# XiaoshuiHuang/GMF

Hardware: AMD Instinct MI355X
Metric: correspondences/sec (whole node) (higher is better)
Workload: dtype f32 (split-fp16 MFMA operands, fp32 accumulate; the cross products of the attention's two contractions, S = K Q'^T and O = P V, on block-scaled e4m3 operands wherever the device-side score guard allows)

## Files before the change

gmf_amd/csrc/enc_common.hpp:

```cpp
#pragma once
#include "mfma_core.hpp"
#include "launchers.hpp"

namespace gmf {

constexpr int C = 128;
constexpr int CF = C / 2;
constexpr int DH = 64;
constexpr int DHF = DH / 2;
constexpr int FFH = 512;
constexpr int kWavesPerWG = 4;

GMF_DEVINL void load_vec_block(float (&v)[16], const float* __restrict__ vec, int mb, int h) {
  const float4* p = reinterpret_cast<const float4*>(vec + 32 * mb) + h;
#pragma unroll
  for (int q = 0; q < 4; ++q) {
    const float4 t = p[2 * q];
    v[4 * q + 0] = t.x; v[4 * q + 1] = t.y; v[4 * q + 2] = t.z; v[4 * q + 3] = t.w;
  }
}

GMF_DEVINL void store_block_p32(float* __restrict__ tile_base, int mb, const float (&t)[16], int lane) {
  float4* p = reinterpret_cast<float4*>(tile_base) + (4 * mb) * 64 + lane;
#pragma unroll
  for (int q = 0; q < 4; ++q) p[q * 64] = make_float4(t[4 * q + 0], t[4 * q + 1], t[4 * q + 2], t[4 * q + 3]);
}

GMF_DEVINL void load_block_p32(float (&t)[16], const float* __restrict__ tile_base, int mb, int lane) {
  const float4* p = reinterpret_cast<const float4*>(tile_base) + (4 * mb) * 64 + lane;
#pragma unroll
  for (int q = 0; q < 4; ++q) {
    const float4 v = p[q * 64];
    t[4 * q + 0] = v.x; t[4 * q + 1] = v.y; t[4 * q + 2] = v.z; t[4 * q + 3] = v.w;
  }
}

GMF_DEVINL void store_block_timg(float* __restrict__ tile_base, int db, const f32x16& a, float bias, int lane) {
  float4* p = reinterpret_cast<float4*>(tile_base) + (4 * db) * 64 + lane;
#pragma unroll
  for (int q = 0; q < 4; ++q)
    p[q * 64] = make_float4(a[4 * q + 0] + bias, a[4 * q + 1] + bias, a[4 * q + 2] + bias, a[4 * q + 3] + bias);
}

GMF_DEVINL void store_block_h2(float* __restrict__ tile_base, int blk, const float (&t)[16], int lane) {
  f16x8* base = reinterpret_cast<f16x8*>(tile_base);
#pragma unroll
  for (int half = 0; half < 2; ++half) {
    f16x8 hi, lo;
    split8h(&t[8 * half], hi, lo);
    const int slot = 2 * blk + half;
    base[(0 * 8 + slot) * 64 + lane] = hi;
    base[(1 * 8 + slot) * 64 + lane] = lo;
  }
}

GMF_DEVINL void store_block_v8(float* __restrict__ tile_base, int db, const float (&t)[16], int lane, unsigned& scale_word) {
  f16x8* base = reinterpret_cast<f16x8*>(tile_base);
  float mx = 0.f;
#pragma unroll
  for (int r = 0; r < 16; ++r) mx = __builtin_fmaxf(mx, __builtin_fabsf(t[r]));
  mx = xhalf_max_swap(mx);
  const int e = (int)((__float_as_uint(mx) >> 23) & 0xffu);
  const int sb = max(e - 7, 105);
  const float s_hi = __uint_as_float((unsigned)sb << 23), s_lo = __uint_as_float((unsigned)(sb - 11) << 23);
  scale_word |= (unsigned)((lane & 32) ? sb : sb - 11) << (8 * db);
  i32x4 v8, l8;
#pragma unroll
  for (int half = 0; half < 2; ++half) {
    f16x8 hi;
#pragma unroll
    for (int j = 0; j < 8; j += 2) {
      const float x0 = t[8 * half + j], x1 = t[8 * half + j + 1];
      const f32x2 x = {x0, x1};
      const f16x2 hh = __builtin_convertvector(x, f16x2);
      const f32x2 rl = resid2h(hh, x0, x1);
      hi[j] = hh[0]; hi[j + 1] = hh[1];
      const int w = 2 * half + (j >> 2);
      if (j & 2) { v8[w] = cvt2_fp8_f32<true>(v8[w], x0, x1, s_hi); l8[w] = cvt2_fp8_f32<true>(l8[w], rl[0], rl[1], s_lo); }
      else { v8[w] = cvt2_fp8_f32<false>(0, x0, x1, s_hi); l8[w] = cvt2_fp8_f32<false>(0, rl[0], rl[1], s_lo); }
    }
    base[(0 * 8 + 2 * db + half) * 64 + lane] = hi;
  }
  reinterpret_cast<i32x4*>(tile_base)[(1 * 8 + 2 * db) * 64 + lane] = l8;
  reinterpret_cast<i32x4*>(tile_base)[(1 * 8 + 2 * db + 1) * 64 + lane] = v8;
}

GMF_DEVINL void q_planes8(const f16x8& h0, const f16x8& l0, const f16x8& h1, const f16x8& l1, int cb, int lane, i32x8& out,
                          unsigned& scale_word) {
  float q[16], ql[16];
#pragma unroll
  for (int e = 0; e < 8; ++e) {
    ql[e] = (float)l0[e]; q[e] = (float)h0[e] + ql[e];
    ql[8 + e] = (float)l1[e]; q[8 + e] = (float)h1[e] + ql[8 + e];
  }
  float mx = 0.f;
#pragma unroll
  for (int r = 0; r < 16; ++r) mx = __builtin_fmaxf(mx, __builtin_fabsf(q[r]));
  mx = xhalf_max_swap(mx);
  const int e = (int)((__float_as_uint(mx) >> 23) & 0xffu);
  const int sb = max(e - 7, 105);
  const float s_hi = __uint_as_float((unsigned)sb << 23), s_lo = __uint_as_float((unsigned)(sb - 11) << 23);
  scale_word |= (unsigned)((lane & 32) ? sb - 11 : sb) << (8 * cb);
#pragma unroll
  for (int w = 0; w < 4; ++w) {
    int a = cvt2_fp8_f32<false>(0, q[4 * w], q[4 * w + 1], s_hi);
    out[w] = cvt2_fp8_f32<true>(a, q[4 * w + 2], q[4 * w + 3], s_hi);
    int b = cvt2_fp8_f32<false>(0, ql[4 * w], ql[4 * w + 1], s_lo);
    out[4 + w] = cvt2_fp8_f32<true>(b, ql[4 * w + 2], ql[4 * w + 3], s_lo);
  }
}

GMF_DEVINL bool pv_planes_on(const unsigned* __restrict__ v_scale, const PvGuard& g, int pair) {
  if (!v_scale) return false;
  if (!g.stat) return true;
// ... 284 lines not shown
```

gmf_amd/csrc/encoder_h2.hip:

```cpp
#include <algorithm>
#include <cstdlib>
#include "enc_common.hpp"
#include "enc_ff.hpp"
#include "launchers.hpp"

namespace gmf {

#ifndef GMF_H2_RING
#define GMF_H2_RING 2
#endif
constexpr int kRing = GMF_H2_RING;

template <int MODE>
GMF_DEVINL void front_h2_body(float* lds, const int bx, const int pair, const int zsel_in, const float* __restrict__ in,
                              const float* __restrict__ wst, const float* __restrict__ vecs, float* __restrict__ f_out,
                              float* __restrict__ q_out, float* __restrict__ k_out, float* __restrict__ v_out, int N, int tiles,
                              const PairTab* __restrict__ ptab = nullptr, unsigned* __restrict__ v_scale = nullptr,
                              const PvGuard guard = {}) {
  const int lane = threadIdx.x & 63, h = lane >> 5, i = lane & 31;
  const int wave = __builtin_amdgcn_readfirstlane(threadIdx.x >> 6);
  const size_t row0 = pair_row0(ptab, pair, N);
  N = pair_rows(ptab, pair, N);
  const int tiles_p = ptab ? (N + 31) >> 5 : tiles;
  if (bx * kWavesPerWG >= tiles_p) return;
// ... 623 lines not shown
  else if (PART != 2) dma_vec(front_vec + C, lvec_p, 3 * C, wave, kWavesPerWG, lane);
  if (PART != 1) {
    dma_vec(attn_vec, lvec_a, 7 * C, wave, kWavesPerWG, lane);
    dma_vec(ff_vec, lvec_f, 3 * C + 2 * FFH, wave, kWavesPerWG, lane);
    LcpeHalo<CF>::issue(pair_base, tile, tiles_p, halo, lane);
  }
  StageRing<4> ss;
  if (KVF && PART == 1) ss.init(lds, wave, lane, kvf_wst, 4);
  else if (KVF && QSKIP) ss.init(lds, wave, lane, attn_wst, 2, ctx_img + (size_t)pair * ttiles * kStageFloats, ttiles, attn_wst + 2 * kStageFloats, 2);
  else if (KVF) ss.init(lds, wave, lane, kvf_wst, 4, attn_wst, 2, ctx_img + (size_t)pair * ttiles * kStageFloats, ttiles, attn_wst + 2 * kStageFloats, 2);
  else if (PART == 0) ss.init(lds, wave, lane, front_wst + (QSKIP ? 8 : 4) * kStageFloats, QSKIP ? 8 : 12, attn_wst, 2,
                         ctx_img + (size_t)pair * ttiles * kStageFloats, ttiles, attn_wst + 2 * kStageFloats, 2);
  else if (PART == 1) ss.init(lds, wave, lane, front_wst + 4 * kStageFloats, 12);
  else ss.init(lds, wave, lane, attn_wst, 2, ctx_img + (size_t)pair * ttiles * kStageFloats, ttiles, attn_wst + 2 * kStageFloats, 2);

  float f[CF];
  if (PART != 2) {
    FragH2<8> fx;
    load_frag_p32<CF>(f, f_in + toff, lane);
    fx.set(f);
    ss.prime();
    const bool v8 = pv_planes_on(v_scale, guard, pair);
    unsigned* const sw_tile = v_scale ? v_scale + ((size_t)pair * tiles + tile) * 128 + lane : nullptr;
    unsigned ksw = 0, vsw = 0;
    if (KVF) {
      asm volatile("s_waitcnt vmcnt(12)" ::: "memory");
      __syncthreads();
      float* const mt = lds + 3 * kStageFloats + wave * 1024;
#pragma unroll
      for (int mb = 0; mb < 4; ++mb) {
        float t[16], td[16];
#pragma unroll
        for (int r = 0; r < 16; ++r) t[r] = f[16 * mb + r];
        if (v8) store_block_v8(k_out + toff, mb, t, lane, ksw);
        else store_block_h2(k_out + toff, mb, t, lane);
#pragma unroll
        for (int r = 0; r < 16; ++r) mt[i * 32 + (frag_feature(r, h) ^ i)] = t[r];
        asm volatile("s_waitcnt lgkmcnt(0)" ::: "memory");
#pragma unroll
        for (int r = 0; r < 16; ++r) { const int kk = frag_feature(r, h); td[r] = mt[kk * 32 + (i ^ kk)]; }
        asm volatile("s_waitcnt lgkmcnt(0)" ::: "memory");
        if (v8) store_block_v8(v_out + toff, mb, td, lane, vsw);
        else store_block_h2(v_out + toff, mb, td, lane);
      }
      if (v_scale) { sw_tile[0] = vsw; sw_tile[64] = ksw; }
      if (!QSKIP) {
#pragma unroll
        for (int mb = 0; mb < 4; ++mb) {
          const f16x8* lw = as_h2(ss.acquire());
          f32x16 acc = zero16();
          mma_wx_h2n<8, NP>(acc, lw, fx);
          float t[16], bb[16];
          load_vec_block(bb, lvec_p, mb, h);
#pragma unroll
          for (int r = 0; r < 16; ++r) t[r] = fmaf(acc[r], kH2Inv, bb[r]);
          store_block_h2(q_out + toff, mb, t, lane);
        }
      }
    }
#pragma unroll
    for (int which = (KVF ? 2 : QSKIP ? 1 : 0); which < 2; ++which) {
      float* dst = (which == 0 ? q_out : k_out) + toff;
#pragma unroll
      for (int mb = 0; mb < 4; ++mb) {
        constexpr int kYounger[4] = {8, 12, 16, 20};
        const int sidx = 4 * (which - (QSKIP ? 1 : 0)) + mb;
        const f16x8* lw = as_h2(PART == 1 ? ss.acquire()
                                : sidx == 0 ? ss.acquire_counted<kYounger[0]>() : sidx == 1 ? ss.acquire_counted<kYounger[1]>()
                                : sidx == 2 ? ss.acquire_counted<kYounger[2]>() : ss.acquire_counted<kYounger[3]>());
        f32x16 acc = zero16();
        mma_wx_h2n<8, NP>(acc, lw, fx);
        float t[16], bb[16];
        load_vec_block(bb, lvec_p + which * C, mb, h);
#pragma unroll
        for (int r = 0; r < 16; ++r) t[r] = fmaf(acc[r], kH2Inv, bb[r]);
// ... 15 lines not shown
    }
    if (v_scale && !KVF) { sw_tile[0] = vsw; sw_tile[64] = ksw; }
  }

  if (PART == 1) {
    asm volatile("s_waitcnt vmcnt(0)" ::: "memory");
    return;
  }
  if (PART == 2) ss.prime();
  f32x16 x1a[4];
  {
    FragH2<4> qx;
    {
      float xp[CF];
      if (PART == 2) load_frag_p32<CF>(xp, f_in + toff, lane);
      else {
#pragma unroll
        for (int k = 0; k < CF; ++k) xp[k] = f[k];
      }
      if (PART == 2) {
        asm volatile("s_waitcnt vmcnt(0)" ::: "memory");
        __syncthreads();
      }
      LcpeHalo<CF>::apply(xp, halo, lvec_a, tile * 32 + i, N, lane);
      {
        FragH2<8> nx;
        {
          float xn[CF];
          layernorm_frag<CF>(xn, xp, lvec_a + 4 * C, lvec_a + 5 * C, h);
          nx.set(xn);
        }
#pragma unroll
        for (int mb = 0; mb < 2; ++mb) {
          const f16x8* lw = as_h2((KVF && QSKIP && PART == 0) ? ss.acquire_counted<40>() : ss.acquire());
          f32x16 acc = zero16();
          mma_wx_h2n<8, NP>(acc, lw, nx);
          float t[16];
#pragma unroll
          for (int r = 0; r < 16; ++r) t[r] = acc[r] * kH2Inv;
          qx.set_block(mb, t);
        }
      }
#pragma unroll
      for (int mb = 0; mb < 4; ++mb) {
        float b[16];
        load_vec_block(b, lvec_a + 6 * C, mb, h);
#pragma unroll
        for (int r = 0; r < 16; ++r) x1a[mb][r] = (xp[16 * mb + r] + b[r]) * 256.0f;
      }
    }
    f32x16 oacc[2];
    oacc[0] = zero16(); oacc[1] = zero16();
    float m_run = -INFINITY, l_half = 0.f;
    for (int t = 0; t < ttiles; ++t) {
      const f16x8* lk = as_h2(ss.acquire());
      const f16x8* lv = lk + 2 * 4 * 64;
      f32x16 sc = zero16();
      mma_wx_h2n<4, NP>(sc, lk, qx);
      float x[16];
      float mx = -INFINITY;
      if (t + 1 < ttiles) {
#pragma unroll
        for (int r = 0; r < 16; ++r) { x[r] = sc[r]; mx = fmaxf(mx, sc[r]); }
      } else {
        const int jbase = t * 32 + 4 * h;
#pragma unroll
        for (int r = 0; r < 16; ++r) {
// ... 271 lines not shown
```

gmf_amd/csrc/encoder_kernels.hip:

```cpp
#include <algorithm>
#include <type_traits>
#include "enc_common.hpp"
#include "enc_ff.hpp"

namespace gmf {

template <int MODE>
__global__ void __launch_bounds__(256, 2)
k_front(const float* __restrict__ in, const float* __restrict__ wst, const float* __restrict__ vecs,
        float* __restrict__ f_out, float* __restrict__ q_out, float* __restrict__ k_out,
        float* __restrict__ v_out, int N, int tiles) {
  __shared__ __attribute__((aligned(16))) float lds[2 * kStageFloats];
  const int lane = threadIdx.x & 63, wave = threadIdx.x >> 6, h = lane >> 5, i = lane & 31;
  const int pair = blockIdx.y;
  const int tile_raw = blockIdx.x * kWavesPerWG + wave;
  const bool active = tile_raw < tiles;
  const int tile = active ? tile_raw : tiles - 1;
  const size_t toff = ((size_t)pair * tiles + tile) * (32 * C);

  constexpr bool FIRST = (MODE == 1);
  StageStream ss;
  if (MODE == 2) ss.init(lds, lds + kStageFloats, wave, kWavesPerWG, lane, wst + 4 * kStageFloats, 12);
  else ss.init(lds, lds + kStageFloats, wave, kWavesPerWG, lane, wst, 16);
  ss.prime();
// ... 526 lines not shown

struct AttnItem { int item, ks; bool split, valid; };
GMF_DEVINL AttnItem attn_item(int L, int n_items, int n_full, int ksplits) {
  const int chunk = n_items >> 3, rem = n_items & 7, xcd = L & 7, kth = L >> 3;
  const int start = (xcd < rem) ? xcd * (chunk + 1) : rem * (chunk + 1) + (xcd - rem) * chunk;
  const int items = chunk + (xcd < rem ? 1 : 0);
  const int nf = min(n_full, items);
  if (kth < nf) return AttnItem{start + kth, 0, false, true};
  const int j = kth - nf, r = j / ksplits;
  return AttnItem{start + nf + r, j - r * ksplits, true, nf + r < items};
}

constexpr float kInvU16 = 1.0f / 65535.0f;
template <int NPROD = 3, int CFMT = 0, bool PVF8 = false, bool FOLD = false>
GMF_DEVINL void scattn_h2p_body(float* lds, const int bid, const float* __restrict__ q_img, const float* __restrict__ k_img,
                                const float* __restrict__ v_img, const float* __restrict__ fus, const float* __restrict__ wst,
                                const float* __restrict__ vecs, float* out, int N, int tiles, int wgs_per_pair,
                                const float* __restrict__ c_dense, int n_items, int n_full, int ksplits,
                                float* __restrict__ part_o, float* __restrict__ part_ml, const float* __restrict__ next_wst,
                                const float* __restrict__ next_bias, const PairTab* __restrict__ ptab = nullptr,
                                const unsigned* __restrict__ v_scale = nullptr,
                                const float* qf_img = nullptr, const float* __restrict__ qw_wst = nullptr,
                                const float* __restrict__ qw_bias = nullptr,
                                unsigned* __restrict__ stat_next = nullptr,
                                const float* __restrict__ kvf_vec = nullptr) {
  static_assert(!PVF8 || NPROD == 3, "the fp8 cross products belong to the three-product form");
  static_assert(!FOLD || NPROD == 3, "the folded form belongs to the parity kernels");
  constexpr int WAVES = 4;
  float* const ldsK = lds;
  float* const ldsV = lds + 2 * kStageFloats;
  const int lane = threadIdx.x & 63, h = lane >> 5;
  const int wave = __builtin_amdgcn_readfirstlane(threadIdx.x >> 6);
  const unsigned lane_off16 = lane * 16;
  const AttnItem it = attn_item(bid, n_items, n_full, ksplits);
  if (!it.valid) return;
  const bool split = it.split;
  const int ks = it.ks;
  const int slot = it.item / wgs_per_pair, qblock = it.item - slot * wgs_per_pair;
  const int pair = ptab ? ptab[slot].ord : slot;
  if (ptab) N = ptab[pair].n;
  const int tiles_p = ptab ? (N + 31) >> 5 : tiles;
  if (qblock * WAVES >= tiles_p) return;
  const int t_begin = split ? (tiles_p * ks) / ksplits : 0;
  const int t_end = split ? (tiles_p * (ks + 1)) / ksplits : tiles_p;
  const int tile_raw = qblock * WAVES + wave;
  const bool active = tile_raw < tiles_p;
  const int tile = active ? tile_raw : tiles_p - 1;
  const size_t pbase = (size_t)pair * tiles;
  const size_t toff = (pbase + tile) * (32 * C);

  f16x8 qh[8], ql[8];
  float beta = 0.f;
  auto fold_beta = [&](const float (&fq)[CF]) {
    float uv[CF], bs = 0.f;
    load_vec_frag<CF>(uv, kvf_vec, h);
#pragma unroll
    for (int e = 0; e < CF; ++e) bs = fmaf(fq[e], uv[e], bs);
    beta = xhalf_sum(bs) + kvf_vec[C];
  };
  if (NPROD == 3 && qw_wst) {
    FragH2<8> fx;
    {
      float fq[CF];
      load_frag_p32<CF>(fq, qf_img + toff, lane);
      fx.set(fq);
      if (FOLD) fold_beta(fq);
// ... 89 lines not shown
  auto mma_n = [&](f32x16& acc, f16x8 ah, f16x8 al, f16x8 bh, f16x8 bl) {
    if (NPROD == 3) mma3(acc, ah, al, bh, bl);
    else acc = mfma_h16(ah, bh, acc);
  };
  auto to_planes2 = [&](float x0, float x1, f16x8& hi, f16x8& lo, int j) {
    if (NPROD == 3) split2h(x0, x1, hi, lo, j);
    else { const f32x2 xx = {x0, x1}; const f16x2 hh = __builtin_convertvector(xx, f16x2); hi[j] = hh[0]; hi[j + 1] = hh[1]; }
  };
  auto planes_f8 = [&](const f16x8& hi, const f16x8& lo, const int j, const int kp, i32x8& pb, float& ls_h, float& ls_l) {
    const f16x2 hh = {hi[j], hi[j + 1]}, ll = {lo[j], lo[j + 1]};
    const f16x2 ones = {(_Float16)1.0f, (_Float16)1.0f};
    const int w = kp >> 1;
    if (kp & 1) {
      pb[w] = cvt2_fp8_f16<true>(pb[w], hh, 4.0f);
      pb[4 + w] = cvt2_fp8_f16<true>(pb[4 + w], ll, 0x1p-10f);
      ls_l = __builtin_amdgcn_fdot2(dec2_fp8_f16<true>(pb[4 + w], 0x1p-10f), ones, ls_l, false);
    } else {
      int d0, d1;
      asm("" : "=v"(d0), "=v"(d1));
      pb[w] = cvt2_fp8_f16<false>(d0, hh, 4.0f);
      pb[4 + w] = cvt2_fp8_f16<false>(d1, ll, 0x1p-10f);
      ls_l = __builtin_amdgcn_fdot2(dec2_fp8_f16<false>(pb[4 + w], 0x1p-10f), ones, ls_l, false);
    }
    ls_h = __builtin_amdgcn_fdot2(hh, ones, ls_h, false);
    asm volatile("" : "+v"(ls_h), "+v"(ls_l));
  };
  const float* gk = k_img + pbase * (size_t)kStageFloats;
  const float* gv = v_img + pbase * (size_t)kStageFloats;
  constexpr int kPiecesPerWave = ((NPROD == 3) ? 16 : 8) / WAVES;
  auto issue16k = [&](const float* g, float* l) {
#pragma unroll
    for (int q = 0; q < kPiecesPerWave; ++q) dma_piece_1k_s(g + (wave + WAVES * q) * 256, l + (wave + WAVES * q) * 256, lane_off16);
  };
  auto issueK = [&](int t) { issue16k(gk + (size_t)t * kStageFloats, ldsK + (t & 1) * kStageFloats); };
  auto issueV = [&](int t) { issue16k(gv + (size_t)t * kStageFloats, ldsV + (t & 1) * kStageFloats); };

  f32x16 oacc[4];
#pragma unroll
  for (int db = 0; db < 4; ++db) oacc[db] = zero16();
  float m_run = -INFINITY, l_half = 0.f;

  issueK(t_begin);
  if (t_begin + 1 < t_end) issueK(t_begin + 1);
  issueV(t_begin);
  fetch_c(t_begin);
  asm volatile("s_waitcnt vmcnt(0)" ::: "memory");
  __syncthreads();
  f32x16 s_a = s_start(), s_b;
  auto s_cross8 = [&](f32x16 acc, const f16x8* lkt, const int cb, const unsigned kscale) -> f32x16 {
    const i32x4* l8 = reinterpret_cast<const i32x4*>(lkt);
    const i32x4 a_lo = l8[(1 * 8 + 2 * cb) * 64], a_hi = l8[(1 * 8 + 2 * cb + 1) * 64];
    const i32x8 ka = {a_lo[0], a_lo[1], a_lo[2], a_lo[3], a_hi[0], a_hi[1], a_hi[2], a_hi[3]};
    return mfma_f8s2(ka, qb[cb], acc, cb, (int)kscale, (int)qsw);
  };
  if (active) {
    const f16x8* lk = reinterpret_cast<const f16x8*>(ldsK + (t_begin & 1) * kStageFloats) + lane;
    if (PVF8) {
      const unsigned ks0 = vsrow[(size_t)t_begin * 128 + 64];
#pragma unroll
      for (int s = 0; s < 8; ++s) s_a = mfma_h16(lk[(0 * 8 + s) * 64], qh[s], s_a);
#pragma unroll
      for (int cb = 0; cb < 4; ++cb) s_a = s_cross8(s_a, lk, cb, ks0);
    } else {
#pragma unroll
      for (int s = 0; s < 8; ++s) mma_n(s_a, lk[(0 * 8 + s) * 64], lk[(1 * 8 + s) * 64], qh[s], ql[s]);
    }
  }

  auto tile_top = [&](const int t, const f32x16& s_cur, float (&x)[16], float& mx) {
    asm volatile("s_waitcnt vmcnt(0)" ::: "memory");
    __syncthreads();
    if (PVF8) vsw = vsw_next;
#pragma unroll
    for (int r = 0; r < 16; r += 2) {
      x[r] = score(r, s_cur[r]);
      x[r + 1] = score(r + 1, s_cur[r + 1]);
      mx = __builtin_fmaxf(mx, __builtin_fmaxf(x[r], x[r + 1]));
    }
    __builtin_amdgcn_sched_barrier(0);
    if (t + 1 < t_end) fetch_c(t + 1);
    __builtin_amdgcn_sched_barrier(0);
  };
  auto issue_piece = [&](const int t, const int q) {
    if ((q & 3) >= kPiecesPerWave) return;
    if (q < 4) {
      if (t + 2 < t_end) dma_piece_1k_s(gk + (size_t)(t + 2) * kStageFloats + (wave + WAVES * q) * 256,
                                        ldsK + (t & 1) * kStageFloats + (wave + WAVES * q) * 256, lane_off16);
    } else {
      dma_piece_1k_s(gv + (size_t)(t + 1) * kStageFloats + (wave + WAVES * (q - 4)) * 256,
                     ldsV + ((t + 1) & 1) * kStageFloats + (wave + WAVES * (q - 4)) * 256, lane_off16);
    }
  };
  auto issue_k4 = [&](const int t) {
    if (t + 2 < t_end && (NPROD == 3 || wave < 2))
      dma_4k_s(gk + (size_t)(t + 2) * kStageFloats + wave * 1024, ldsK + (t & 1) * kStageFloats + wave * 1024, lane_off16);
  };
  auto issue_v4 = [&](const int t) {
    if (NPROD == 3 || wave < 2)
      dma_4k_s(gv + (size_t)(t + 1) * kStageFloats + wave * 1024, ldsV + ((t + 1) & 1) * kStageFloats + wave * 1024, lane_off16);
  };
  auto rescale = [&](const bool moved, const float alpha) {
    if (__any(moved)) {
#pragma unroll
      for (int db = 0; db < 4; ++db)
#pragma unroll
        for (int r = 0; r < 16; ++r) oacc[db][r] *= alpha;
    }
  };
  auto tile_step = [&](const int t, const f32x16& s_cur, f32x16& s_next) {
    float x[16];
    float mx = -INFINITY, m_off = 0.f, alpha = 1.f, ls = 0.f;
    tile_top(t, s_cur, x, mx);
    const f16x8* lv = reinterpret_cast<const f16x8*>(ldsV + (t & 1) * kStageFloats) + lane;
    const f16x8* lk = reinterpret_cast<const f16x8*>(ldsK + ((t + 1) & 1) * kStageFloats) + lane;
    bool moved = false;
    f16x8 ph0, pl0, ph1, pl1;
    {
      mx = xhalf_max_swap(mx);
      if (CFMT == 2) mx *= kInvU16;
      const float m_new = __builtin_fmaxf(m_run, mx);
      moved = m_new > m_run;
      alpha = __builtin_amdgcn_exp2f(m_run - m_new);
      m_run = m_new;
      m_off = m_new - 10.0f;
      rescale(moved, alpha);
    }
    s_next = s_start();
    {
      f16x8 kh = lk[0], kl = kh;
      if (NPROD == 3) kl = lk[8 * 64];
      f16x8 kh_n = kh, kl_n = kl;
// ... 23 lines not shown
      }
    }
    {
      f16x8 vh = lv[0], vl = vh;
      if (NPROD == 3) vl = lv[8 * 64];
      f16x8 vh_n = vh, vl_n = vl;
#pragma unroll
      for (int u = 0; u < 24; ++u) {
        const int s2 = u / 12, db = (u % 12) / 3, pr = u % 3;
        if (pr == 0 && u < 21) {
          const int un = u + 3, slot = 2 * ((un % 12) / 3) + un / 12;
          vh_n = lv[(0 * 8 + slot) * 64]; if (NPROD == 3) vl_n = lv[(1 * 8 + slot) * 64];
        }
        if (NPROD == 3 || pr == 2) oacc[db] = mma3_part(pr, oacc[db], vh, vl, s2 ? ph1 : ph0, s2 ? pl1 : pl0);
        if (pr == 2) { vh = vh_n; vl = vl_n; }
        if (u < 2) {
          const int j = 4 + 2 * u;
          to_planes2(x[8 + j], x[8 + j + 1], ph1, pl1, j);
        }
        if (u >= 3 && u < 11) issue_piece(t, u - 3);
        __builtin_amdgcn_sched_barrier(0);
      }
    }
    l_half = fmaf(l_half, alpha, ls);
  };
  constexpr float kLazy = 5.0f;
  auto tile_step_f8 = [&](const int t, const f32x16& s_cur, f32x16& s_next) {
    float x[16];
    float mx = -INFINITY, m_off = 0.f, alpha = 1.f, ls = 0.f, ls_l = 0.f;
    asm volatile("s_waitcnt vmcnt(0)" ::: "memory");
    __syncthreads();
    vsw = vsw_next;
    ksw = ksw_next;
    const f16x8* lv = reinterpret_cast<const f16x8*>(ldsV + (t & 1) * kStageFloats) + lane;
    const f16x8* lk = reinterpret_cast<const f16x8*>(ldsK + ((t + 1) & 1) * kStageFloats) + lane;
    f16x8 ph0, pl0, ph1, pl1;
    i32x8 pb;
    f16x8 vr[3];
    auto hslot = [](int u) { return (0 * 8 + 2 * (u & 3) + (u >> 2)) * 64; };
    s_next = s_start();
    {
      const i32x4* lk8 = reinterpret_cast<const i32x4*>(lk);
      f16x8 kh = lk[0];
      f16x8 kh_n = kh;
      i32x4 k8a = lk8[(1 * 8) * 64], k8b = lk8[(1 * 8 + 1) * 64];
#pragma unroll
      for (int u = 0; u < 24; ++u) {
        const int s = u / 3, pr = u % 3;
        if (pr == 0 && s < 7) kh_n = lk[(0 * 8 + s + 1) * 64];
        if (pr == 2) s_next = mfma_h16(kh, qh[s], s_next);
        if (pr == 0 && (s & 1)) {
          const int cb = s >> 1;
          const i32x8 ka = {k8a[0], k8a[1], k8a[2], k8a[3], k8b[0], k8b[1], k8b[2], k8b[3]};
          s_next = mfma_f8s2(ka, qb[cb], s_next, cb, (int)ksw, (int)qsw);
          if (cb < 3) { k8a = lk8[(1 * 8 + 2 * cb + 2) * 64]; k8b = lk8[(1 * 8 + 2 * cb + 3) * 64]; }
        }
        if (pr == 2) kh = kh_n;
        if (u < 4) {
#pragma unroll
          for (int r = 4 * u; r < 4 * u + 4; r += 2) {
            x[r] = score(r, s_cur[r]);
            x[r + 1] = score(r + 1, s_cur[r + 1]);
            mx = __builtin_fmaxf(mx, __builtin_fmaxf(x[r], x[r + 1]));
          }
        }
        if (u == 3) {
          __builtin_amdgcn_sched_barrier(0);
          if (t + 1 < t_end) fetch_c(t + 1);
          __builtin_amdgcn_sched_barrier(0);
          mx = xhalf_max_swap(mx);
          if (CFMT == 2) mx *= kInvU16;
          const bool moved = mx > m_run + kLazy;
          const float m_new = moved ? mx : m_run;
          alpha = __builtin_amdgcn_exp2f(m_run - m_new);
          m_run = m_new;
          m_off = m_new - (10.0f - kLazy);
          rescale(moved, alpha);
        }
        if (u >= 4 && u < 20) x[u - 4] = expo(x[u - 4], m_off);
        if (u >= 6 && u <= 18 && (u & 1) == 0) {
          const int k = (u - 6) >> 1;
          if (k < 4) split2h(x[2 * k], x[2 * k + 1], ph0, pl0, 2 * k);
          else split2h(x[2 * k], x[2 * k + 1], ph1, pl1, 2 * k - 8);
        }
        if (u == 20) split2h(x[14], x[15], ph1, pl1, 6);
        if (u == 16) issue_k4(t);
        if (u == 23) issue_v4(t);
        if (u >= 21) vr[u - 21] = lv[hslot(u - 21)];
        __builtin_amdgcn_sched_barrier(0);
      }
    }
    {
      const i32x4* lv8 = reinterpret_cast<const i32x4*>(lv);
      i32x4 fa[2][2];
#pragma unroll
      for (int u = 0; u < 12; ++u) {
        if (u < 8) {
          const int s2 = u >> 2, db = u & 3;
          oacc[db] = mfma_h16(vr[u % 3], s2 ? ph1 : ph0, oacc[db]);
          if (u + 3 < 8) vr[u % 3] = lv[hslot(u + 3)];
          if (u == 4 || u == 6) { const int fd = (u - 4) >> 1; fa[fd][0] = lv8[(1 * 8 + 2 * fd) * 64]; fa[fd][1] = lv8[(1 * 8 + 2 * fd + 1) * 64]; }
          planes_f8(u < 4 ? ph0 : ph1, u < 4 ? pl0 : pl1, 2 * (u & 3), u, pb, ls, ls_l);
        } else {
          const int db = u - 8;
          const i32x4 a_lo = fa[db & 1][0], a_hi = fa[db & 1][1];
          const i32x8 va = {a_lo[0], a_lo[1], a_lo[2], a_lo[3], a_hi[0], a_hi[1], a_hi[2], a_hi[3]};
          oacc[db] = mfma_f8s(va, pb, oacc[db], db, (int)vsw, psc);
          if (db < 2) { fa[db & 1][0] = lv8[(1 * 8 + 2 * db + 4) * 64]; fa[db & 1][1] = lv8[(1 * 8 + 2 * db + 5) * 64]; }
        }
        __builtin_amdgcn_sched_barrier(0);
      }
    }
    l_half = fmaf(l_half, alpha, ls + ls_l);
  };
  auto tile_last = [&](const int t, const f32x16& s_cur) {
    float x[16];
    float mx = -INFINITY, ls = 0.f;
    tile_top(t, s_cur, x, mx);
    const f16x8* lv = reinterpret_cast<const f16x8*>(ldsV + (t & 1) * kStageFloats) + lane;
    const int jbase = t * 32 + 4 * h;
    mx = -INFINITY;
#pragma unroll
    for (int r = 0; r < 16; ++r) {
      const int jl = 8 * (r >> 2) + (r & 3);
      x[r] = (jbase + jl < N) ? x[r] : -INFINITY;
      mx = __builtin_fmaxf(mx, x[r]);
    }
    mx = xhalf_max_swap(mx);
    if (CFMT == 2) mx *= kInvU16;
    const float m_new = __builtin_fmaxf(m_run, mx);
    const bool moved = m_new > m_run;
    const float alpha = __builtin_amdgcn_exp2f(m_run - m_new);
    m_run = m_new;
    const float m_off = m_new - (PVF8 ? 10.0f - kLazy : 10.0f);
#pragma unroll
    for (int r = 0; r < 16; ++r) { x[r] = expo(x[r], m_off); if (!PVF8) ls += x[r]; }
    rescale(moved, alpha);
    if (PVF8) {
      i32x8 pb;
      float ls_l = 0.f;
#pragma unroll
      for (int s2 = 0; s2 < 2; ++s2) {
        f16x8 ph, pl;
        split8h(&x[8 * s2], ph, pl);
#pragma unroll
        for (int j = 0; j < 8; j += 2) planes_f8(ph, pl, j, 4 * s2 + (j >> 1), pb, ls, ls_l);
#pragma unroll
        for (int db = 0; db < 4; ++db) oacc[db] = mfma_h16(lv[(0 * 8 + 2 * db + s2) * 64], ph, oacc[db]);
      }
      ls += ls_l;
      const i32x4* lv8 = reinterpret_cast<const i32x4*>(lv);
#pragma unroll
      for (int db = 0; db < 4; ++db) {
        const i32x4 a_lo = lv8[(1 * 8 + 2 * db) * 64], a_hi = lv8[(1 * 8 + 2 * db + 1) * 64];
        const i32x8 va = {a_lo[0], a_lo[1], a_lo[2], a_lo[3], a_hi[0], a_hi[1], a_hi[2], a_hi[3]};
        oacc[db] = mfma_f8s(va, pb, oacc[db], db, (int)vsw, psc);
      }
    } else {
#pragma unroll
    for (int s2 = 0; s2 < 2; ++s2) {
      f16x8 ph, pl;
      split8h(&x[8 * s2], ph, pl);
#pragma unroll
      for (int db = 0; db < 4; ++db) {
        const int slot = 2 * db + s2;
        mma_n(oacc[db], lv[(0 * 8 + slot) * 64], lv[(1 * 8 + slot) * 64], ph, pl);
      }
    }
    }
    l_half = fmaf(l_half, alpha, ls);
  };
  if (!active) {
    for (int t = t_begin; t < t_end; ++t) {
      asm volatile("s_waitcnt vmcnt(0)" ::: "memory");
      __syncthreads();
      if (t + 1 < t_end) {
        if (PVF8) { issue_k4(t); issue_v4(t); }
        else {
#pragma unroll
          for (int q = 0; q < 8; ++q) issue_piece(t, q);
        }
      }
    }
  } else {
    int t = t_begin;
    if (PVF8) {
      for (; t + 2 < t_end; t += 2) {
// ... 1132 lines not shown
```

gmf_amd/csrc/mfma_core.hpp:

```cpp
#pragma once
#include <hip/hip_runtime.h>
#include <stdint.h>

#include "launchers.hpp"

#define GMF_DEVINL __device__ __forceinline__

namespace gmf {

GMF_DEVINL int pair_rows(const PairTab* pt, int pair, int N) { return pt ? pt[pair].n : N; }
GMF_DEVINL size_t pair_row0(const PairTab* pt, int pair, int N) { return pt ? (size_t)pt[pair].row0 : (size_t)pair * N; }

typedef float f32x16 __attribute__((ext_vector_type(16)));
typedef float f32x4 __attribute__((ext_vector_type(4)));

constexpr int kWave = 64;
constexpr int kTileRows = 32;
constexpr int kStageFloats = 4096;

GMF_DEVINL f32x16 mfma32(float a, float b, f32x16 c) {
  return __builtin_amdgcn_mfma_f32_32x32x2f32(a, b, c, 0, 0, 0);
}

typedef float f32x2 __attribute__((ext_vector_type(2)));
// ... 200 lines not shown
  const float rstd = rsqrtf(xhalf_sum(v) * (1.0f / (2 * KF)) + 1e-5f);
  const float4* pg = reinterpret_cast<const float4*>(gamma) + h;
  const float4* pb = reinterpret_cast<const float4*>(beta) + h;
#pragma unroll
  for (int g = 0; g < KF / 4; ++g) {
    const float4 ga = pg[2 * g], be = pb[2 * g];
    y[4 * g + 0] = fmaf((x[4 * g + 0] - mu) * rstd, ga.x, be.x);
    y[4 * g + 1] = fmaf((x[4 * g + 1] - mu) * rstd, ga.y, be.y);
    y[4 * g + 2] = fmaf((x[4 * g + 2] - mu) * rstd, ga.z, be.z);
    y[4 * g + 3] = fmaf((x[4 * g + 3] - mu) * rstd, ga.w, be.w);
  }
}

GMF_DEVINL void dma_piece_1k(const float* __restrict__ gsrc_piece, float* lds_piece, int lane) {
  __builtin_amdgcn_global_load_lds(
      (const void __attribute__((address_space(1)))*)(gsrc_piece + lane * 4),
      (void __attribute__((address_space(3)))*)(lds_piece), 16, 0, 0);
}

GMF_DEVINL void dma_piece_1k_s(const float* __restrict__ gsrc_piece_uniform, float* lds_piece, unsigned lane_off16) {
  unsigned keep;
  const unsigned lds_dst = (unsigned)(uintptr_t)(void __attribute__((address_space(3)))*)(lds_piece);
  asm volatile("s_mov_b32 %0, m0\n\ts_mov_b32 m0, %3\n\ts_nop 0\n\tglobal_load_lds_dwordx4 %1, %2\n\ts_mov_b32 m0, %0"
               : "=&s"(keep) : "v"(lane_off16), "s"(gsrc_piece_uniform), "s"(lds_dst) : "memory");
}

GMF_DEVINL void dma_4k_s(const float* __restrict__ gsrc_uniform, float* lds_dst_base, unsigned lane_off16) {
  unsigned keep;
  const unsigned lds_dst = (unsigned)(uintptr_t)(void __attribute__((address_space(3)))*)(lds_dst_base);
  asm volatile("s_mov_b32 %0, m0\n\ts_mov_b32 m0, %3\n\ts_nop 0\n\t"
               "global_load_lds_dwordx4 %1, %2\n\tglobal_load_lds_dwordx4 %1, %2 offset:1024\n\t"
               "global_load_lds_dwordx4 %1, %2 offset:2048\n\tglobal_load_lds_dwordx4 %1, %2 offset:3072\n\ts_mov_b32 m0, %0"
               : "=&s"(keep) : "v"(lane_off16), "s"(gsrc_uniform), "s"(lds_dst) : "memory");
}

GMF_DEVINL void dma_vec(const float* __restrict__ gsrc, float* lds_dst, int n_floats, int wave, int n_waves, int lane) {
  for (int p = wave; p * 256 < n_floats; p += n_waves)
    if (p * 256 + lane * 4 < n_floats) dma_piece_1k(gsrc + p * 256, lds_dst + p * 256, lane);
}

GMF_DEVINL void dma_issue(const float* __restrict__ gsrc, float* lds_dst, int n_pieces, int wave, int n_waves, int lane) {
  for (int p = wave; p < n_pieces; p += n_waves) dma_piece_1k(gsrc + p * 256, lds_dst + p * 256, lane);
}

struct StageStream {
  const float* seg_ptr[3];
  int seg_end[3];
  int stage_floats = kStageFloats;
  float* buf0;
  float* buf1;
  int issued;
  int consumed;
  int total;
  int wave, n_waves, lane;

  GMF_DEVINL void init(float* b0, float* b1, int wave_, int n_waves_, int lane_, const float* p0, int n0,
                       const float* p1 = nullptr, int n1 = 0, const float* p2 = nullptr, int n2 = 0) {
    seg_ptr[0] = p0; seg_ptr[1] = p1; seg_ptr[2] = p2;
    seg_end[0] = n0; seg_end[1] = n0 + n1; seg_end[2] = n0 + n1 + n2;
    total = seg_end[2];
    buf0 = b0; buf1 = b1; issued = 0; consumed = 0;
    wave = wave_; n_waves = n_waves_; lane = lane_;
  }
  GMF_DEVINL void issue_one() {
    if (issued < total) {
      const float* g;
// ... 72 lines not shown
```

Before: 11.10 million.

## Share one fp16 hi plane for K and V via transposing LDS reads

```diff
diff --git a/gmf_amd/csrc/enc_common.hpp b/gmf_amd/csrc/enc_common.hpp
--- a/gmf_amd/csrc/enc_common.hpp
+++ b/gmf_amd/csrc/enc_common.hpp
@@ -1,6 +1,7 @@
 #pragma once
 #include "mfma_core.hpp"
 #include "launchers.hpp"
+#include "kv_share_layout.hpp"
 
 namespace gmf {
 
@@ -54,6 +55,8 @@
   }
 }
 
+enum { kHiFrag = 0, kHiShared = 1, kHiNone = 2 };
+template <int HI = kHiFrag>
 GMF_DEVINL void store_block_v8(float* __restrict__ tile_base, int db, const float (&t)[16], int lane, unsigned& scale_word) {
   f16x8* base = reinterpret_cast<f16x8*>(tile_base);
   float mx = 0.f;
@@ -79,7 +82,8 @@
       if (j & 2) { v8[w] = cvt2_fp8_f32<true>(v8[w], x0, x1, s_hi); l8[w] = cvt2_fp8_f32<true>(l8[w], rl[0], rl[1], s_lo); }
       else { v8[w] = cvt2_fp8_f32<false>(0, x0, x1, s_hi); l8[w] = cvt2_fp8_f32<false>(0, rl[0], rl[1], s_lo); }
     }
-    base[(0 * 8 + 2 * db + half) * 64 + lane] = hi;
+    if (HI == kHiFrag) base[(0 * 8 + 2 * db + half) * 64 + lane] = hi;
+    else if (HI == kHiShared) base[kvshare::row_read_addr(lane, 2 * db + half) / 16] = hi;
   }
   reinterpret_cast<i32x4*>(tile_base)[(1 * 8 + 2 * db) * 64 + lane] = l8;
   reinterpret_cast<i32x4*>(tile_base)[(1 * 8 + 2 * db + 1) * 64 + lane] = v8;
diff --git a/gmf_amd/csrc/encoder_h2.hip b/gmf_amd/csrc/encoder_h2.hip
--- a/gmf_amd/csrc/encoder_h2.hip
+++ b/gmf_amd/csrc/encoder_h2.hip
@@ -679,7 +679,7 @@
         float t[16], td[16];
 #pragma unroll
         for (int r = 0; r < 16; ++r) t[r] = f[16 * mb + r];
-        if (v8) store_block_v8(k_out + toff, mb, t, lane, ksw);
+        if (v8) store_block_v8<kHiShared>(k_out + toff, mb, t, lane, ksw);
         else store_block_h2(k_out + toff, mb, t, lane);
 #pragma unroll
         for (int r = 0; r < 16; ++r) mt[i * 32 + (frag_feature(r, h) ^ i)] = t[r];
@@ -687,7 +687,7 @@
 #pragma unroll
         for (int r = 0; r < 16; ++r) { const int kk = frag_feature(r, h); td[r] = mt[kk * 32 + (i ^ kk)]; }
         asm volatile("s_waitcnt lgkmcnt(0)" ::: "memory");
-        if (v8) store_block_v8(v_out + toff, mb, td, lane, vsw);
+        if (v8) store_block_v8<kHiNone>(v_out + toff, mb, td, lane, vsw);
         else store_block_h2(v_out + toff, mb, td, lane);
       }
       if (v_scale) { sw_tile[0] = vsw; sw_tile[64] = ksw; }
@@ -769,7 +769,7 @@
         }
 #pragma unroll
         for (int mb = 0; mb < 2; ++mb) {
-          const f16x8* lw = as_h2((KVF && QSKIP && PART == 0) ? ss.acquire_counted<40>() : ss.acquire());
+          const f16x8* lw = as_h2((KVF && QSKIP && PART == 0) ? ss.acquire_counted<32>() : ss.acquire());
           f32x16 acc = zero16();
           mma_wx_h2n<8, NP>(acc, lw, nx);
           float t[16];
diff --git a/gmf_amd/csrc/encoder_kernels.hip b/gmf_amd/csrc/encoder_kernels.hip
--- a/gmf_amd/csrc/encoder_kernels.hip
+++ b/gmf_amd/csrc/encoder_kernels.hip
@@ -582,6 +582,36 @@
   const int lane = threadIdx.x & 63, h = lane >> 5;
   const int wave = __builtin_amdgcn_readfirstlane(threadIdx.x >> 6);
   const unsigned lane_off16 = lane * 16;
+  constexpr bool SHARE = PVF8 && FOLD;
+  constexpr int kPlaneFloats = kStageFloats / 2;
+  float* const ldsH = lds;
+  float* const ldsKx = lds + 2 * kStageFloats;
+  float* const ldsVx = lds + 3 * kStageFloats;
+  const unsigned lds_h0 = (unsigned)(uintptr_t)(void __attribute__((address_space(3)))*)(lds);
+  const unsigned row_b0 = lds_h0 + kvshare::row_read_addr(lane, 0), row_b1 = lds_h0 + kvshare::row_read_addr(lane, 1);
+  const unsigned tr_b0 = lds_h0 + kvshare::tr_read_addr(lane, 0, h), tr_b1 = lds_h0 + kvshare::tr_read_addr(lane, 0, 2 + h);
+  struct PlaneAddr { unsigned a, b; };
+  auto plane_addr = [&](const int t, const unsigned b0, const unsigned b1) -> PlaneAddr {
+    PlaneAddr pa{b0 + (t & 3) * kvshare::kPlaneBytes, b1 + (t & 3) * kvshare::kPlaneBytes};
+    if (SHARE) asm("" : "+v"(pa.a), "+v"(pa.b));
+    return pa;
+  };
+  auto k_addr = [&](const int t) { return plane_addr(t, row_b0, row_b1); };
+  auto v_addr = [&](const int t) { return plane_addr(t, tr_b0, tr_b1); };
+  auto k_rows = [&](const int t, const PlaneAddr& ka, const int s) -> f16x8 {
+    if (SHARE) return lds_read_f16x8(((s & 1) ? ka.b : ka.a) + 512 * (s >> 1));
+    return (reinterpret_cast<const f16x8*>(ldsK + (t & 1) * kStageFloats) + lane)[(0 * 8 + s) * 64];
+  };
+  auto v_cols = [&](const int t, const PlaneAddr& va, const int db, const int s2) -> f16x8 {
+    if (SHARE) return lds_read_tr16x8(va.a + 512 * db + 4096 * s2, va.b + 512 * db + 4096 * s2);
+    return (reinterpret_cast<const f16x8*>(ldsV + (t & 1) * kStageFloats) + lane)[(0 * 8 + 2 * db + s2) * 64];
+  };
+  auto k_cross = [&](const int t) -> const i32x4* {
+    return reinterpret_cast<const i32x4*>(SHARE ? ldsKx + (t & 1) * kPlaneFloats : ldsK + (t & 1) * kStageFloats + kPlaneFloats) + lane;
+  };
+  auto v_cross = [&](const int t) -> const i32x4* {
+    return reinterpret_cast<const i32x4*>(SHARE ? ldsVx + (t & 1) * kPlaneFloats : ldsV + (t & 1) * kStageFloats + kPlaneFloats) + lane;
+  };
   const AttnItem it = attn_item(bid, n_items, n_full, ksplits);
   if (!it.valid) return;
   const bool split = it.split;
@@ -737,8 +767,20 @@
 #pragma unroll
     for (int q = 0; q < kPiecesPerWave; ++q) dma_piece_1k_s(g + (wave + WAVES * q) * 256, l + (wave + WAVES * q) * 256, lane_off16);
   };
-  auto issueK = [&](int t) { issue16k(gk + (size_t)t * kStageFloats, ldsK + (t & 1) * kStageFloats); };
-  auto issueV = [&](int t) { issue16k(gv + (size_t)t * kStageFloats, ldsV + (t & 1) * kStageFloats); };
+  auto issue8k = [&](const float* g, float* l) {
+#pragma unroll
+    for (int q = 0; q < 2; ++q) dma_piece_1k_s(g + (wave + WAVES * q) * 256, l + (wave + WAVES * q) * 256, lane_off16);
+  };
+  auto issueK = [&](int t) {
+    if (SHARE) {
+      issue8k(gk + (size_t)t * kStageFloats, ldsH + (t & 3) * kPlaneFloats);
+      issue8k(gk + (size_t)t * kStageFloats + kPlaneFloats, ldsKx + (t & 1) * kPlaneFloats);
+    } else issue16k(gk + (size_t)t * kStageFloats, ldsK + (t & 1) * kStageFloats);
+  };
+  auto issueV = [&](int t) {
+    if (SHARE) issue8k(gv + (size_t)t * kStageFloats + kPlaneFloats, ldsVx + (t & 1) * kPlaneFloats);
+    else issue16k(gv + (size_t)t * kStageFloats, ldsV + (t & 1) * kStageFloats);
+  };
 
   f32x16 oacc[4];
 #pragma unroll
@@ -752,9 +794,8 @@
   asm volatile("s_waitcnt vmcnt(0)" ::: "memory");
   __syncthreads();
   f32x16 s_a = s_start(), s_b;
-  auto s_cross8 = [&](f32x16 acc, const f16x8* lkt, const int cb, const unsigned kscale) -> f32x16 {
-    const i32x4* l8 = reinterpret_cast<const i32x4*>(lkt);
-    const i32x4 a_lo = l8[(1 * 8 + 2 * cb) * 64], a_hi = l8[(1 * 8 + 2 * cb + 1) * 64];
+  auto s_cross8 = [&](f32x16 acc, const i32x4* l8, const int cb, const unsigned kscale) -> f32x16 {
+    const i32x4 a_lo = l8[(2 * cb) * 64], a_hi = l8[(2 * cb + 1) * 64];
     const i32x8 ka = {a_lo[0], a_lo[1], a_lo[2], a_lo[3], a_hi[0], a_hi[1], a_hi[2], a_hi[3]};
     return mfma_f8s2(ka, qb[cb], acc, cb, (int)kscale, (int)qsw);
   };
@@ -762,10 +803,11 @@
     const f16x8* lk = reinterpret_cast<const f16x8*>(ldsK + (t_begin & 1) * kStageFloats) + lane;
     if (PVF8) {
       const unsigned ks0 = vsrow[(size_t)t_begin * 128 + 64];
-#pragma unroll
-      for (int s = 0; s < 8; ++s) s_a = mfma_h16(lk[(0 * 8 + s) * 64], qh[s], s_a);
-#pragma unroll
-      for (int cb = 0; cb < 4; ++cb) s_a = s_cross8(s_a, lk, cb, ks0);
+      const PlaneAddr ka = k_addr(t_begin);
+#pragma unroll
+      for (int s = 0; s < 8; ++s) s_a = mfma_h16(k_rows(t_begin, ka, s), qh[s], s_a);
+#pragma unroll
+      for (int cb = 0; cb < 4; ++cb) s_a = s_cross8(s_a, k_cross(t_begin), cb, ks0);
     } else {
 #pragma unroll
       for (int s = 0; s < 8; ++s) mma_n(s_a, lk[(0 * 8 + s) * 64], lk[(1 * 8 + s) * 64], qh[s], ql[s]);
@@ -797,11 +839,17 @@
     }
   };
   auto issue_k4 = [&](const int t) {
-    if (t + 2 < t_end && (NPROD == 3 || wave < 2))
+    if (SHARE) {
+      if (t + 2 < t_end)
+        dma_4k_s(gk + (size_t)(t + 2) * kStageFloats + wave * 1024,
+                 wave < 2 ? ldsH + ((t + 2) & 3) * kPlaneFloats + wave * 1024 : ldsKx + (t & 1) * kPlaneFloats + (wave - 2) * 1024, lane_off16);
+    } else if (t + 2 < t_end && (NPROD == 3 || wave < 2))
       dma_4k_s(gk + (size_t)(t + 2) * kStageFloats + wave * 1024, ldsK + (t & 1) * kStageFloats + wave * 1024, lane_off16);
   };
   auto issue_v4 = [&](const int t) {
-    if (NPROD == 3 || wave < 2)
+    if (SHARE)
+      dma_2k_s(gv + (size_t)(t + 1) * kStageFloats + kPlaneFloats + wave * 512, ldsVx + ((t + 1) & 1) * kPlaneFloats + wave * 512, lane_off16);
+    else if (NPROD == 3 || wave < 2)
       dma_4k_s(gv + (size_t)(t + 1) * kStageFloats + wave * 1024, ldsV + ((t + 1) & 1) * kStageFloats + wave * 1024, lane_off16);
   };
   auto rescale = [&](const bool moved, const float alpha) {
@@ -891,28 +939,28 @@
     __syncthreads();
     vsw = vsw_next;
     ksw = ksw_next;
-    const f16x8* lv = reinterpret_cast<const f16x8*>(ldsV + (t & 1) * kStageFloats) + lane;
-    const f16x8* lk = reinterpret_cast<const f16x8*>(ldsK + ((t + 1) & 1) * kStageFloats) + lane;
     f16x8 ph0, pl0, ph1, pl1;
     i32x8 pb;
     f16x8 vr[3];
-    auto hslot = [](int u) { return (0 * 8 + 2 * (u & 3) + (u >> 2)) * 64; };
+    PlaneAddr va{0u, 0u};
+    auto v_hi = [&](const int u) { return v_cols(t, va, u & 3, u >> 2); };
     s_next = s_start();
     {
-      const i32x4* lk8 = reinterpret_cast<const i32x4*>(lk);
-      f16x8 kh = lk[0];
+      const i32x4* lk8 = k_cross(t + 1);
+      const PlaneAddr ka = k_addr(t + 1);
+      f16x8 kh = k_rows(t + 1, ka, 0);
       f16x8 kh_n = kh;
-      i32x4 k8a = lk8[(1 * 8) * 64], k8b = lk8[(1 * 8 + 1) * 64];
+      i32x4 k8a = lk8[0], k8b = lk8[64];
 #pragma unroll
       for (int u = 0; u < 24; ++u) {
         const int s = u / 3, pr = u % 3;
-        if (pr == 0 && s < 7) kh_n = lk[(0 * 8 + s + 1) * 64];
+        if (pr == 0 && s < 7) kh_n = k_rows(t + 1, ka, s + 1);
         if (pr == 2) s_next = mfma_h16(kh, qh[s], s_next);
         if (pr == 0 && (s & 1)) {
           const int cb = s >> 1;
           const i32x8 ka = {k8a[0], k8a[1], k8a[2], k8a[3], k8b[0], k8b[1], k8b[2], k8b[3]};
           s_next = mfma_f8s2(ka, qb[cb], s_next, cb, (int)ksw, (int)qsw);
-          if (cb < 3) { k8a = lk8[(1 * 8 + 2 * cb + 2) * 64]; k8b = lk8[(1 * 8 + 2 * cb + 3) * 64]; }
+          if (cb < 3) { k8a = lk8[(2 * cb + 2) * 64]; k8b = lk8[(2 * cb + 3) * 64]; }
         }
         if (pr == 2) kh = kh_n;
         if (u < 4) {
@@ -945,27 +993,28 @@
         if (u == 20) split2h(x[14], x[15], ph1, pl1, 6);
         if (u == 16) issue_k4(t);
         if (u == 23) issue_v4(t);
-        if (u >= 21) vr[u - 21] = lv[hslot(u - 21)];
+        if (u == 21) va = v_addr(t);
+        if (u >= 21) vr[u - 21] = v_hi(u - 21);
         __builtin_amdgcn_sched_barrier(0);
       }
     }
     {
-      const i32x4* lv8 = reinterpret_cast<const i32x4*>(lv);
+      const i32x4* lv8 = v_cross(t);
       i32x4 fa[2][2];
 #pragma unroll
       for (int u = 0; u < 12; ++u) {
         if (u < 8) {
           const int s2 = u >> 2, db = u & 3;
           oacc[db] = mfma_h16(vr[u % 3], s2 ? ph1 : ph0, oacc[db]);
-          if (u + 3 < 8) vr[u % 3] = lv[hslot(u + 3)];
-          if (u == 4 || u == 6) { const int fd = (u - 4) >> 1; fa[fd][0] = lv8[(1 * 8 + 2 * fd) * 64]; fa[fd][1] = lv8[(1 * 8 + 2 * fd + 1) * 64]; }
+          if (u + 3 < 8) vr[u % 3] = v_hi(u + 3);
+          if (u == 4 || u == 6) { const int fd = (u - 4) >> 1; fa[fd][0] = lv8[(2 * fd) * 64]; fa[fd][1] = lv8[(2 * fd + 1) * 64]; }
           planes_f8(u < 4 ? ph0 : ph1, u < 4 ? pl0 : pl1, 2 * (u & 3), u, pb, ls, ls_l);
         } else {
           const int db = u - 8;
           const i32x4 a_lo = fa[db & 1][0], a_hi = fa[db & 1][1];
           const i32x8 va = {a_lo[0], a_lo[1], a_lo[2], a_lo[3], a_hi[0], a_hi[1], a_hi[2], a_hi[3]};
           oacc[db] = mfma_f8s(va, pb, oacc[db], db, (int)vsw, psc);
-          if (db < 2) { fa[db & 1][0] = lv8[(1 * 8 + 2 * db + 4) * 64]; fa[db & 1][1] = lv8[(1 * 8 + 2 * db + 5) * 64]; }
+          if (db < 2) { fa[db & 1][0] = lv8[(2 * db + 4) * 64]; fa[db & 1][1] = lv8[(2 * db + 5) * 64]; }
         }
         __builtin_amdgcn_sched_barrier(0);
       }
@@ -998,6 +1047,7 @@
     if (PVF8) {
       i32x8 pb;
       float ls_l = 0.f;
+      const PlaneAddr va = v_addr(t);
 #pragma unroll
       for (int s2 = 0; s2 < 2; ++s2) {
         f16x8 ph, pl;
@@ -1005,13 +1055,13 @@
 #pragma unroll
         for (int j = 0; j < 8; j += 2) planes_f8(ph, pl, j, 4 * s2 + (j >> 1), pb, ls, ls_l);
 #pragma unroll
-        for (int db = 0; db < 4; ++db) oacc[db] = mfma_h16(lv[(0 * 8 + 2 * db + s2) * 64], ph, oacc[db]);
+        for (int db = 0; db < 4; ++db) oacc[db] = mfma_h16(v_cols(t, va, db, s2), ph, oacc[db]);
       }
       ls += ls_l;
-      const i32x4* lv8 = reinterpret_cast<const i32x4*>(lv);
+      const i32x4* lv8 = v_cross(t);
 #pragma unroll
       for (int db = 0; db < 4; ++db) {
-        const i32x4 a_lo = lv8[(1 * 8 + 2 * db) * 64], a_hi = lv8[(1 * 8 + 2 * db + 1) * 64];
+        const i32x4 a_lo = lv8[(2 * db) * 64], a_hi = lv8[(2 * db + 1) * 64];
         const i32x8 va = {a_lo[0], a_lo[1], a_lo[2], a_lo[3], a_hi[0], a_hi[1], a_hi[2], a_hi[3]};
         oacc[db] = mfma_f8s(va, pb, oacc[db], db, (int)vsw, psc);
       }
diff --git a/gmf_amd/csrc/kv_share_layout.hpp b/gmf_amd/csrc/kv_share_layout.hpp
--- /dev/null
+++ b/gmf_amd/csrc/kv_share_layout.hpp
@@ -0,0 +1,20 @@
+#pragma once
+
+namespace gmf {
+namespace kvshare {
+
+constexpr unsigned kPlaneBytes = 32 * 128 * 2;
+
+constexpr unsigned off(unsigned row, unsigned ch) {
+  return 2048u * (row >> 3) + 512u * (ch >> 2) + 64u * (row & 7u) + 16u * ((ch & 3u) ^ ((row >> 2) & 3u));
+}
+
+constexpr unsigned row_read_addr(unsigned lane, unsigned s) { return off(lane & 31u, 2u * s + (lane >> 5)); }
+
+constexpr unsigned tr_read_addr(unsigned lane, unsigned db, unsigned kg) {
+  const unsigned j = lane & 15u, q = j >> 2, p = j & 3u, gb = (lane >> 4) & 1u;
+  return off(4u * kg + q, 4u * db + 2u * gb + (p & 1u)) + 8u * (p >> 1);
+}
+
+}
+}
diff --git a/gmf_amd/csrc/mfma_core.hpp b/gmf_amd/csrc/mfma_core.hpp
--- a/gmf_amd/csrc/mfma_core.hpp
+++ b/gmf_amd/csrc/mfma_core.hpp
@@ -256,6 +256,27 @@
                "global_load_lds_dwordx4 %1, %2\n\tglobal_load_lds_dwordx4 %1, %2 offset:1024\n\t"
                "global_load_lds_dwordx4 %1, %2 offset:2048\n\tglobal_load_lds_dwordx4 %1, %2 offset:3072\n\ts_mov_b32 m0, %0"
                : "=&s"(keep) : "v"(lane_off16), "s"(gsrc_uniform), "s"(lds_dst) : "memory");
+}
+
+GMF_DEVINL void dma_2k_s(const float* __restrict__ gsrc_uniform, float* lds_dst_base, unsigned lane_off16) {
+  unsigned keep;
+  const unsigned lds_dst = (unsigned)(uintptr_t)(void __attribute__((address_space(3)))*)(lds_dst_base);
+  asm volatile("s_mov_b32 %0, m0\n\ts_mov_b32 m0, %3\n\ts_nop 0\n\t"
+               "global_load_lds_dwordx4 %1, %2\n\tglobal_load_lds_dwordx4 %1, %2 offset:1024\n\ts_mov_b32 m0, %0"
+               : "=&s"(keep) : "v"(lane_off16), "s"(gsrc_uniform), "s"(lds_dst) : "memory");
+}
+
+typedef __fp16 h16x4_tr __attribute__((__vector_size__(8)));
+GMF_DEVINL f16x8 lds_read_tr16x8(unsigned addr_a, unsigned addr_b) {
+  typedef _Float16 f16x4v __attribute__((ext_vector_type(4)));
+  const f16x4v a = __builtin_bit_cast(f16x4v, __builtin_amdgcn_ds_read_tr16_b64_v4f16(
+      (h16x4_tr __attribute__((address_space(3)))*)(uintptr_t)addr_a));
+  const f16x4v b = __builtin_bit_cast(f16x4v, __builtin_amdgcn_ds_read_tr16_b64_v4f16(
+      (h16x4_tr __attribute__((address_space(3)))*)(uintptr_t)addr_b));
+  return __builtin_shufflevector(a, b, 0, 1, 2, 3, 4, 5, 6, 7);
+}
+GMF_DEVINL f16x8 lds_read_f16x8(unsigned addr) {
+  return *(const f16x8 __attribute__((address_space(3)))*)(uintptr_t)addr;
 }
 
 GMF_DEVINL void dma_vec(const float* __restrict__ gsrc, float* lds_dst, int n_floats, int wave, int n_waves, int lane) {
```

Result: faster. 11.22 million (median of 6 runs) (+1.1%).
